# aicip/Cross-Scale-MAE

Measured on AMD Instinct MI355X. Metric: pretrain images/sec ViT-B/16 224^2 two-scale, higher is better.
Workload: dtype bf16; 1 GPU; MAE_ViT_MsLdCeCd ViT-B/16, 224^2 two-scale crops, mask 0.75, AdamW, full optimizer step; loss=mse, batch_per_gpu=128, global_batch=128, parallelism=dp1, headline_config=True

## Files before the change

### cross-scale-mae_amd/csrc/attention.hip

```cpp
#include "common.h"
#include <cstdlib>

#define LOG2E 1.4426950408889634f
#define LN2 0.6931471805599453f

template <int HD> struct AttnLds { static constexpr int STRIDE = (HD + 8) * 2; };

template <int HD, int TP>
__device__ __forceinline__ void stage_head(char* dst, const bf16_t* src, long long row0, int ld, int col0, int T, int hd) {
  constexpr int CH = HD / 8;
  for (int e = threadIdx.x; e < TP * CH; e += blockDim.x) {
    int r = e / CH, c = e - r * CH;
    uint4 v = make_uint4(0, 0, 0, 0);
    if (r < T && c * 8 < hd) v = *reinterpret_cast<const uint4*>(src + (row0 + r) * ld + col0 + c * 8);
    *reinterpret_cast<uint4*>(dst + r * AttnLds<HD>::STRIDE + c * 16) = v;
  }
}

template <int HD, int TP, int NT, int NM>
struct HeadStager {
  static constexpr int CH = HD / 8, IT = (TP * CH + NT - 1) / NT;
  uint4 v[NM][IT];
  __device__ __forceinline__ void load(int m, const bf16_t* src, long long row0, int ld, int col0, int T, int hd) {
#pragma unroll
    for (int i = 0; i < IT; ++i) {
      const int e = threadIdx.x + i * NT, r = e / CH, c = e - r * CH;
      v[m][i] = make_uint4(0, 0, 0, 0);
      if (e < TP * CH && r < T && c * 8 < hd) v[m][i] = *reinterpret_cast<const uint4*>(src + (row0 + r) * ld + col0 + c * 8);
    }
  }
  __device__ __forceinline__ void store(int m, char* dst) {
#pragma unroll
    for (int i = 0; i < IT; ++i) {
      const int e = threadIdx.x + i * NT, r = e / CH, c = e - r * CH;
      if (e < TP * CH) *reinterpret_cast<uint4*>(dst + r * AttnLds<HD>::STRIDE + c * 16) = v[m][i];
    }
  }
};

template <int HD>
__device__ __forceinline__ s8_t frag_rows(const char* img, int row0, int ks, int t, int g) {
  return *reinterpret_cast<const s8_t*>(img + (row0 + t) * AttnLds<HD>::STRIDE + (ks * 32 + 8 * g) * 2);
}
template <int HD>
__device__ __forceinline__ s8_t frag_cols_tr(const char* img, int r0, int c0, int t, int g) {
  const char* p = img + (r0 + 4 * g + (t >> 2)) * AttnLds<HD>::STRIDE + (c0 + (t & 3) * 4) * 2;
  s4_t lo = __builtin_amdgcn_ds_read_tr16_b64_v4i16(LDS_PTR(s4_t, p));
  s4_t hi = __builtin_amdgcn_ds_read_tr16_b64_v4i16(LDS_PTR(s4_t, p + 16 * AttnLds<HD>::STRIDE));
  return join_s4(lo, hi);
}
__device__ __forceinline__ s8_t pack_pair(f4_t a, f4_t b) {
  unsigned u0 = pack2bf(a[0], a[1]), u1 = pack2bf(a[2], a[3]), u2 = pack2bf(b[0], b[1]), u3 = pack2bf(b[2], b[3]);
  uint4 u = make_uint4(u0, u1, u2, u3);
  return __builtin_bit_cast(s8_t, u);
}
#define MFMA16(a, b, c) __builtin_amdgcn_mfma_f32_16x16x32_bf16(__builtin_bit_cast(bf8_t, a), __builtin_bit_cast(bf8_t, b), c, 0, 0, 0)

template <int HD>
__device__ __forceinline__ int pair_remap(int bid, int nblk) {
  if (HD * 2 >= 128 || (bid | 15) >= nblk) return bid;
  return (bid & ~15) + 2 * (bid & 7) + ((bid >> 3) & 1);
}

template <int HD, int NKF, bool EMIT = false>
__global__ __launch_bounds__(256) void attn_fwd_bf16(const bf16_t* __restrict__ qkv, bf16_t* __restrict__ out,
                                                     float* __restrict__ lse, int T, int H, int D, int hd, float scale, Fp8Emit em) {
  constexpr int TP = NKF * 16, KS = HD / 32, DF = HD / 16;
  constexpr int QB = (NKF + 3) / 4;
  __shared__ __attribute__((aligned(16))) char smem[2 * TP * AttnLds<HD>::STRIDE];
  char* Ks = smem;
  char* Vs = smem + TP * AttnLds<HD>::STRIDE;
  const int wid = pair_remap<HD>(blockIdx.x, gridDim.x);
  const int b = wid / H, h = wid - b * H;
  const long long row0 = (long long)b * T;
  const int ld = 3 * D;
  const int lane = threadIdx.x & 63, w = threadIdx.x >> 6, t = lane & 15, g = lane >> 4;
  uint4 qraw[QB][KS];
  {
    HeadStager<HD, TP, 256, 2> sg;
    sg.load(0, qkv, row0, ld, D + h * hd, T, hd); sg.load(1, qkv, row0, ld, 2 * D + h * hd, T, hd);
#pragma unroll
    for (int bq = 0; bq < QB; ++bq)
#pragma unroll
      for (int ks = 0; ks < KS; ++ks) {
        const int qr = (w + 4 * bq) * 16 + t, col = ks * 32 + 8 * g;
        qraw[bq][ks] = make_uint4(0, 0, 0, 0);
        if (qr < T && col < hd) qraw[bq][ks] = *reinterpret_cast<const uint4*>(qkv + (row0 + qr) * ld + h * hd + col);
      }
    sg.store(0, Ks); sg.store(1, Vs);
// ... 6 lines not shown
  constexpr int FIRST_PARTIAL = NKF <= 2 ? 0 : (NKF <= 6 ? NKF - 2 : (NKF == 14 ? 6 : 14));
  const int kthr = T - 4 * g;
#pragma unroll
  for (int bq = 0; bq < QB; ++bq) {
    const int qb = w + 4 * bq;
    if (qb >= nqb) break;
    const int q = qb * 16 + t;
    s8_t fq[KS];
#pragma unroll
    for (int ks = 0; ks < KS; ++ks) fq[ks] = __builtin_bit_cast(s8_t, qraw[bq][ks]);
    f4_t s[NKF];
    float m = -INFINITY;
#pragma unroll
    for (int f = 0; f < NKF; ++f) {
      f4_t a = {0.f, 0.f, 0.f, 0.f};
#pragma unroll
      for (int ks = 0; ks < KS; ++ks) a = MFMA16(frag_rows<HD>(Ks, f * 16, ks, t, g), fq[ks], a);
      if (f >= FIRST_PARTIAL) {
#pragma unroll
        for (int r = 0; r < 4; ++r) a[r] = (f * 16 + r >= kthr) ? -INFINITY : a[r];
      }
      m = fmaxf(fmaxf(m, fmaxf(a[0], a[1])), fmaxf(a[2], a[3]));
      s[f] = a;
    }
    m = xrow_max(m);
    m *= c2;
    float l = 0.f;
#pragma unroll
    for (int f = 0; f < NKF; ++f)
#pragma unroll
      for (int r = 0; r < 4; ++r) { float p = __builtin_amdgcn_exp2f(fmaf(s[f][r], c2, -m)); s[f][r] = p; l += p; }
    l = xrow_sum(l);
    const float inv = 1.0f / l;
    s8_t fp[NKF / 2];
#pragma unroll
    for (int s2 = 0; s2 < NKF / 2; ++s2) fp[s2] = pack_pair(s[2 * s2], s[2 * s2 + 1]);
#pragma unroll
    for (int df = 0; df < DF; ++df) {
      f4_t o = {0.f, 0.f, 0.f, 0.f};
#pragma unroll
      for (int s2 = 0; s2 < NKF / 2; ++s2) o = MFMA16(frag_cols_tr<HD>(Vs, 32 * s2, df * 16, t, g), fp[s2], o);
      int d = df * 16 + 4 * g;
      if (q < T && d < hd) {
        const long long at = (row0 + q) * D + h * hd + d;
        st4<bf16_t>(out + at, o * inv);
        if (EMIT) *reinterpret_cast<unsigned*>(em.q + at) = fp8_pack4(round4<bf16_t>(o * inv), qs, qmax, em.fmt, qseen);
      }
    }
    if (g == 0 && q < T) lse[((long long)b * H + h) * T + q] = (m + log2f(l)) * LN2;
  }
  if (EMIT) fp8_emit_amax(em, qseen, threadIdx.x & 63);
}

template <bool EMIT>
__device__ __forceinline__ void st4_dqkv(bf16_t* dqkv, long long at, f4_t v, const Fp8Emit& em, float qs, float qmax, float& qseen) {
  if (!EMIT || dqkv) st4<bf16_t>(dqkv + at, v);
  if (EMIT) *reinterpret_cast<unsigned*>(em.q + at) = fp8_pack4(round4<bf16_t>(v), qs, qmax, em.fmt, qseen);
}
template <int HD, int NKF, bool EMIT = false>
__global__ __launch_bounds__(256) void attn_bwd_bf16(const bf16_t* __restrict__ qkv, const bf16_t* __restrict__ out,
                                                     const bf16_t* __restrict__ dout, const float* __restrict__ lse,
                                                     bf16_t* __restrict__ dqkv, int T, int H, int D, int hd, float scale, Fp8Emit em) {
  constexpr int TP = NKF * 16, KS = HD / 32, DF = HD / 16, IMG = TP * AttnLds<HD>::STRIDE;
  __shared__ __attribute__((aligned(16))) char smem[4 * IMG + 2 * TP * 4];
  char* Qs = smem; char* Ks = smem + IMG; char* Vs = smem + 2 * IMG; char* Gs = smem + 3 * IMG;
  float* lse2 = reinterpret_cast<float*>(smem + 4 * IMG);
  float* dl = lse2 + TP;
  const int wid = pair_remap<HD>(blockIdx.x, gridDim.x);
  const int b = wid / H, h = wid - b * H;
  const long long row0 = (long long)b * T;
  const int ld = 3 * D;
  {
    HeadStager<HD, TP, 256, 4> sg;
    sg.load(0, qkv, row0, ld, h * hd, T, hd); sg.load(1, qkv, row0, ld, D + h * hd, T, hd);
    sg.load(2, qkv, row0, ld, 2 * D + h * hd, T, hd); sg.load(3, dout, row0, D, h * hd, T, hd);
    sg.store(0, Qs); sg.store(1, Ks); sg.store(2, Vs); sg.store(3, Gs);
  }
  for (int r = threadIdx.x; r < TP; r += blockDim.x) {
    float acc = 0.f, l2 = INFINITY;
    if (r < T) {
      l2 = lse[((long long)b * H + h) * T + r] * LOG2E;
      const bf16_t* o = out + (row0 + r) * D + h * hd;
      const bf16_t* gg = dout + (row0 + r) * D + h * hd;
      uint4 ov[HD / 8], gv[HD / 8];
#pragma unroll
      for (int c = 0; c < HD / 8; ++c) {
        ov[c] = c * 8 < hd ? *reinterpret_cast<const uint4*>(o + c * 8) : make_uint4(0, 0, 0, 0);
        gv[c] = c * 8 < hd ? *reinterpret_cast<const uint4*>(gg + c * 8) : make_uint4(0, 0, 0, 0);
      }
#pragma unroll
      for (int c = 0; c < HD / 8; ++c) {
        const unsigned ow[4] = {ov[c].x, ov[c].y, ov[c].z, ov[c].w}, gw[4] = {gv[c].x, gv[c].y, gv[c].z, gv[c].w};
#pragma unroll
        for (int k = 0; k < 4; ++k)
          acc += __uint_as_float(ow[k] << 16) * __uint_as_float(gw[k] << 16) + __uint_as_float(ow[k] & 0xffff0000u) * __uint_as_float(gw[k] & 0xffff0000u);
      }
    }
    lse2[r] = l2; dl[r] = acc;
  }
  __syncthreads();
  const int lane = threadIdx.x & 63, w = threadIdx.x >> 6, t = lane & 15, g = lane >> 4;
  float qmax = 0.f, qseen = 0.f;
  const float qs = EMIT ? fp8_emit_scale(em, lane, qmax) : 1.f;
  const float c2 = scale * LOG2E;
  const int nblk = (T + 15) >> 4;
  for (int qb = w; qb < nblk; qb += 4) {
    const int q = qb * 16 + t;
    s8_t fq[KS], fg[KS];
#pragma unroll
    for (int ks = 0; ks < KS; ++ks) { fq[ks] = frag_rows<HD>(Qs, qb * 16, ks, t, g); fg[ks] = frag_rows<HD>(Gs, qb * 16, ks, t, g); }
    const float my_l2 = lse2[q], my_dl = dl[q];
    s8_t fds[NKF / 2];
    f4_t prev = {0.f, 0.f, 0.f, 0.f};
#pragma unroll
    for (int f = 0; f < NKF; ++f) {
      f4_t a = {0.f, 0.f, 0.f, 0.f}, dp = {0.f, 0.f, 0.f, 0.f};
#pragma unroll
      for (int ks = 0; ks < KS; ++ks) {
        a = MFMA16(frag_rows<HD>(Ks, f * 16, ks, t, g), fq[ks], a);
        dp = MFMA16(frag_rows<HD>(Vs, f * 16, ks, t, g), fg[ks], dp);
      }
      f4_t ds;
#pragma unroll
      for (int r = 0; r < 4; ++r) {
        float p = __builtin_amdgcn_exp2f(a[r] * c2 - my_l2);
        ds[r] = p * (dp[r] - my_dl) * scale;
      }
      if (f & 1) fds[f >> 1] = pack_pair(prev, ds); else prev = ds;
    }
#pragma unroll
    for (int df = 0; df < DF; ++df) {
      f4_t o = {0.f, 0.f, 0.f, 0.f};
#pragma unroll
      for (int s2 = 0; s2 < NKF / 2; ++s2) o = MFMA16(frag_cols_tr<HD>(Ks, 32 * s2, df * 16, t, g), fds[s2], o);
      int d = df * 16 + 4 * g;
      if (q < T && d < hd) st4_dqkv<EMIT>(dqkv, (row0 + q) * ld + h * hd + d, o, em, qs, qmax, qseen);
    }
  }
  for (int kb = w; kb < nblk; kb += 4) {
    const int key = kb * 16 + t;
    s8_t fk[KS], fv[KS];
#pragma unroll
    for (int ks = 0; ks < KS; ++ks) { fk[ks] = frag_rows<HD>(Ks, kb * 16, ks, t, g); fv[ks] = frag_rows<HD>(Vs, kb * 16, ks, t, g); }
    s8_t fp[NKF / 2], fds[NKF / 2];
    f4_t prev_p = {0.f, 0.f, 0.f, 0.f}, prev_ds = {0.f, 0.f, 0.f, 0.f};
#pragma unroll
    for (int f = 0; f < NKF; ++f) {
      f4_t a = {0.f, 0.f, 0.f, 0.f}, dp = {0.f, 0.f, 0.f, 0.f};
#pragma unroll
      for (int ks = 0; ks < KS; ++ks) {
        a = MFMA16(frag_rows<HD>(Qs, f * 16, ks, t, g), fk[ks], a);
        dp = MFMA16(frag_rows<HD>(Gs, f * 16, ks, t, g), fv[ks], dp);
      }
      f4_t l4 = *reinterpret_cast<const f4_t*>(lse2 + f * 16 + 4 * g);
      f4_t d4 = *reinterpret_cast<const f4_t*>(dl + f * 16 + 4 * g);
      f4_t p, ds;
#pragma unroll
      for (int r = 0; r < 4; ++r) {
        p[r] = __builtin_amdgcn_exp2f(a[r] * c2 - l4[r]);
        ds[r] = p[r] * (dp[r] - d4[r]) * scale;
      }
      if (f & 1) { fp[f >> 1] = pack_pair(prev_p, p); fds[f >> 1] = pack_pair(prev_ds, ds); } else { prev_p = p; prev_ds = ds; }
    }
#pragma unroll
    for (int df = 0; df < DF; ++df) {
      f4_t ok = {0.f, 0.f, 0.f, 0.f}, ov = {0.f, 0.f, 0.f, 0.f};
#pragma unroll
      for (int s2 = 0; s2 < NKF / 2; ++s2) {
        ok = MFMA16(frag_cols_tr<HD>(Qs, 32 * s2, df * 16, t, g), fds[s2], ok);
        ov = MFMA16(frag_cols_tr<HD>(Gs, 32 * s2, df * 16, t, g), fp[s2], ov);
      }
      int d = df * 16 + 4 * g;
      if (key < T && d < hd) {
        st4_dqkv<EMIT>(dqkv, (row0 + key) * ld + D + h * hd + d, ok, em, qs, qmax, qseen);
        st4_dqkv<EMIT>(dqkv, (row0 + key) * ld + 2 * D + h * hd + d, ov, em, qs, qmax, qseen);
      }
    }
  }
  if (EMIT) fp8_emit_amax(em, qseen, lane);
}

template <int HD, int NKF>
struct AttnBwd1p {
  static constexpr int NP = NKF / 2, TP = NKF * 16, IMG = TP * AttnLds<HD>::STRIDE, QS = HD + 4;
  static constexpr int XB = 32 * HD * 2;
  static constexpr int LDS = 2 * IMG + TP * QS * 4 + 4 * XB + 2 * TP * 4;
  static constexpr int LDS8 = LDS + 4 * XB;
};
template <int HD>
__device__ __forceinline__ s8_t patch_cols_tr(const char* img, int c0, int t, int g) {
  const char* p = img + (4 * g + (t >> 2)) * (HD * 2) + (c0 + (t & 3) * 4) * 2;
  s4_t lo = __builtin_amdgcn_ds_read_tr16_b64_v4i16(LDS_PTR(s4_t, p));
  s4_t hi = __builtin_amdgcn_ds_read_tr16_b64_v4i16(LDS_PTR(s4_t, p + 16 * HD * 2));
  return join_s4(lo, hi);
}
#ifdef ATTN_TIMING
__device__ unsigned long long g_attn_ts[16];
extern "C" int csmae_debug_attn_ts(unsigned long long* out) { return (int)hipMemcpyFromSymbol(out, HIP_SYMBOL(g_attn_ts), sizeof(g_attn_ts)); }
#define TS(i) do { if (blockIdx.x == 300 && threadIdx.x == 0) g_attn_ts[i] = __builtin_readcyclecounter(); } while (0)
#else
#define TS(i)
#endif
template <int HD, int NKF, bool EMIT = false, int NW = 4>
__global__ __launch_bounds__(NW * 64, NW == 4 ? 2 : 1) void attn_bwd1p_bf16(const bf16_t* __restrict__ qkv, const bf16_t* __restrict__ out,
                                                           const bf16_t* __restrict__ dout, const float* __restrict__ lse,
                                                           bf16_t* __restrict__ dqkv, int T, int H, int D, int hd, float scale, Fp8Emit em) {
  using L = AttnBwd1p<HD, NKF>;
  constexpr int TP = L::TP, NP = L::NP, KS = HD / 32, DF = HD / 16, IMG = L::IMG, QS = L::QS;
  static_assert(NW == 4 || (NW == 8 && NP >= 8), "eight waves need at least eight query pairs for the dQ rotation");
  __shared__ __attribute__((aligned(16))) char smem[NW == 4 ? L::LDS : L::LDS8];
  char* Qs = smem; char* Gs = smem + IMG;
  float* dqa = reinterpret_cast<float*>(smem + 2 * IMG);
  char* xall = smem + 2 * IMG + TP * QS * 4;
  float* lse2 = reinterpret_cast<float*>(xall + NW * L::XB);
  float* dl = lse2 + TP;
  const int wid = pair_remap<HD>(blockIdx.x, gridDim.x);
  const int b = wid / H, h = wid - b * H;
  const long long row0 = (long long)b * T;
  const int ld = 3 * D;
  const int lane = threadIdx.x & 63, w = threadIdx.x >> 6, t = lane & 15, g = lane >> 4;
  float qmax = 0.f, qseen = 0.f;
  const float qs = EMIT ? fp8_emit_scale(em, lane, qmax) : 1.f;
  TS(0);
  HeadStager<HD, TP, NW * 64, 2> sg;
  sg.load(0, qkv, row0, ld, h * hd, T, hd); sg.load(1, dout, row0, D, h * hd, T, hd);
  const int nkp = (T + 31) >> 5;
  uint4 kraw[2][KS], vraw[2][KS];
  auto load_kv = [&](int kp) {
#pragma unroll
    for (int jj = 0; jj < 2; ++jj)
#pragma unroll
      for (int ks = 0; ks < KS; ++ks) {
        const int key = 32 * kp + 16 * jj + t, col = ks * 32 + 8 * g;
        kraw[jj][ks] = make_uint4(0, 0, 0, 0); vraw[jj][ks] = make_uint4(0, 0, 0, 0);
        if (kp < nkp && key < T && col < hd) {
          kraw[jj][ks] = *reinterpret_cast<const uint4*>(qkv + (row0 + key) * ld + D + h * hd + col);
          vraw[jj][ks] = *reinterpret_cast<const uint4*>(qkv + (row0 + key) * ld + 2 * D + h * hd + col);
        }
      }
  };
  load_kv(w);
  for (int e = threadIdx.x; e < TP * QS / 4; e += blockDim.x) reinterpret_cast<f4_t*>(dqa)[e] = f4_t{0.f, 0.f, 0.f, 0.f};
  for (int r = threadIdx.x; r < TP; r += blockDim.x) {
    float acc = 0.f, l2 = INFINITY;
    if (r < T) {
      l2 = lse[((long long)b * H + h) * T + r] * LOG2E;
      const bf16_t* o = out + (row0 + r) * D + h * hd;
      const bf16_t* gg = dout + (row0 + r) * D + h * hd;
      uint4 ov[HD / 8], gv[HD / 8];
#pragma unroll
      for (int c = 0; c < HD / 8; ++c) {
        ov[c] = c * 8 < hd ? *reinterpret_cast<const uint4*>(o + c * 8) : make_uint4(0, 0, 0, 0);
        gv[c] = c * 8 < hd ? *reinterpret_cast<const uint4*>(gg + c * 8) : make_uint4(0, 0, 0, 0);
      }
#pragma unroll
      for (int c = 0; c < HD / 8; ++c) {
        const unsigned ow[4] = {ov[c].x, ov[c].y, ov[c].z, ov[c].w}, gw[4] = {gv[c].x, gv[c].y, gv[c].z, gv[c].w};
#pragma unroll
        for (int k = 0; k < 4; ++k)
          acc += __uint_as_float(ow[k] << 16) * __uint_as_float(gw[k] << 16) + __uint_as_float(ow[k] & 0xffff0000u) * __uint_as_float(gw[k] & 0xffff0000u);
      }
    }
    lse2[r] = l2; dl[r] = acc;
  }
  TS(1);
  sg.store(0, Qs); sg.store(1, Gs);
  const float c2 = scale * LOG2E;
  char* xw = xall + w * L::XB;
  const int nq = (T + 31) >> 5;
  for (int sweep = 0; sweep * NW < nkp; ++sweep) {
    const int kp = sweep * NW + w;
    const bool active = kp < nkp;
    const int k0 = 32 * kp;
    s8_t fk[2][KS], fv[2][KS], kT[DF];
#pragma unroll
    for (int jj = 0; jj < 2; ++jj)
#pragma unroll
      for (int ks = 0; ks < KS; ++ks) {
        const int col = ks * 32 + 8 * g;
        fk[jj][ks] = __builtin_bit_cast(s8_t, kraw[jj][ks]); fv[jj][ks] = __builtin_bit_cast(s8_t, vraw[jj][ks]);
        *reinterpret_cast<uint4*>(xw + (16 * jj + t) * (HD * 2) + col * 2) = kraw[jj][ks];
      }
#pragma unroll
    for (int df = 0; df < DF; ++df) kT[df] = patch_cols_tr<HD>(xw, df * 16, t, g);
    f4_t dk[2][DF], dv[2][DF];
#pragma unroll
    for (int jj = 0; jj < 2; ++jj)
#pragma unroll
      for (int df = 0; df < DF; ++df) { dk[jj][df] = f4_t{0.f, 0.f, 0.f, 0.f}; dv[jj][df] = f4_t{0.f, 0.f, 0.f, 0.f}; }
    TS(2 + 4 * sweep);
    __syncthreads();
    TS(3 + 4 * sweep);
    if ((sweep + 1) * NW < nkp) load_kv((sweep + 1) * NW + w);
    for (int s = 0; s < nq; ++s) {
      int ip = w + s; if (ip >= nq) ip -= nq;
      const int q0 = 32 * ip;
      if (active && w < nq) {
        f4_t p[2][2], ds[2][2];
#pragma unroll
        for (int ii = 0; ii < 2; ++ii) {
          s8_t fq[KS], fg[KS];
#pragma unroll
          for (int ks = 0; ks < KS; ++ks) { fq[ks] = frag_rows<HD>(Qs, q0 + 16 * ii, ks, t, g); fg[ks] = frag_rows<HD>(Gs, q0 + 16 * ii, ks, t, g); }
          const f4_t l4 = *reinterpret_cast<const f4_t*>(lse2 + q0 + 16 * ii + 4 * g);
          const f4_t d4 = *reinterpret_cast<const f4_t*>(dl + q0 + 16 * ii + 4 * g);
#pragma unroll
          for (int jj = 0; jj < 2; ++jj) {
            f4_t a = {0.f, 0.f, 0.f, 0.f}, dp = {0.f, 0.f, 0.f, 0.f};
#pragma unroll
            for (int ks = 0; ks < KS; ++ks) { a = MFMA16(fq[ks], fk[jj][ks], a); dp = MFMA16(fg[ks], fv[jj][ks], dp); }
#pragma unroll
            for (int r = 0; r < 4; ++r) {
              p[ii][jj][r] = __builtin_amdgcn_exp2f(a[r] * c2 - l4[r]);
              ds[ii][jj][r] = p[ii][jj][r] * (dp[r] - d4[r]) * scale;
            }
            uint2 u = make_uint2(pack2bf(ds[ii][jj][0], ds[ii][jj][1]), pack2bf(ds[ii][jj][2], ds[ii][jj][3]));
            *reinterpret_cast<uint2*>(xw + (ii * 2 + jj) * 512 + t * 32 + g * 8) = u;
          }
        }
// ... 15 lines not shown
          f4_t* dst = reinterpret_cast<f4_t*>(dqa + (q0 + 16 * ii + t) * QS + 4 * g);
#pragma unroll
          for (int df = 0; df < DF; ++df) dst[df * 4] = MFMA16(kT[df], sT, dst[df * 4]);
        }
      }
      __syncthreads();
    }
    TS(4 + 4 * sweep);
    if (active) {
#pragma unroll
      for (int jj = 0; jj < 2; ++jj) {
        const int key = k0 + 16 * jj + t;
#pragma unroll
        for (int df = 0; df < DF; ++df) {
          const int d = df * 16 + 4 * g;
          if (key < T && d < hd) {
            st4_dqkv<EMIT>(dqkv, (row0 + key) * ld + D + h * hd + d, dk[jj][df], em, qs, qmax, qseen);
            st4_dqkv<EMIT>(dqkv, (row0 + key) * ld + 2 * D + h * hd + d, dv[jj][df], em, qs, qmax, qseen);
          }
        }
      }
    }
  }
  TS(10);
  for (int e = threadIdx.x; e < T * (HD / 4); e += blockDim.x) {
    const int q = e / (HD / 4), d = (e - q * (HD / 4)) * 4;
    if (d < hd) st4_dqkv<EMIT>(dqkv, (row0 + q) * ld + h * hd + d, *reinterpret_cast<const f4_t*>(dqa + q * QS + d), em, qs, qmax, qseen);
  }
  if (EMIT) fp8_emit_amax(em, qseen, lane);
}

template <int HD, int NKF, bool EMIT = false>
__global__ __launch_bounds__(256, 2) void attn_bwd1p2_bf16(const bf16_t* __restrict__ qkv, const bf16_t* __restrict__ out,
                                                            const bf16_t* __restrict__ dout, const float* __restrict__ lse,
                                                            bf16_t* __restrict__ dqkv, int T, int H, int D, int hd, float scale, Fp8Emit em) {
  using L = AttnBwd1p<HD, NKF>;
  constexpr int TP = L::TP, NP = L::NP, KS = HD / 32, DF = HD / 16, IMG = L::IMG, QS = L::QS;
  static_assert(NP <= 8, "two key pairs per wave cover at most eight");
  constexpr int NPW = NP > 4 ? 2 : 1;
  __shared__ __attribute__((aligned(16))) char smem[L::LDS];
  char* Qs = smem; char* Gs = smem + IMG;
  float* dqa = reinterpret_cast<float*>(smem + 2 * IMG);
  char* xall = smem + 2 * IMG + TP * QS * 4;
  float* lse2 = reinterpret_cast<float*>(xall + 4 * L::XB);
  float* dl = lse2 + TP;
  const int wid = pair_remap<HD>(blockIdx.x, gridDim.x);
  const int b = wid / H, h = wid - b * H;
  const long long row0 = (long long)b * T;
  const int ld = 3 * D;
  const int lane = threadIdx.x & 63, w = threadIdx.x >> 6, t = lane & 15, g = lane >> 4;
  float qmax = 0.f, qseen = 0.f;
  const float qs = EMIT ? fp8_emit_scale(em, lane, qmax) : 1.f;
  TS(0);
  HeadStager<HD, TP, 256, 2> sg;
  sg.load(0, qkv, row0, ld, h * hd, T, hd); sg.load(1, dout, row0, D, h * hd, T, hd);
  const int nkp = (T + 31) >> 5;
  uint4 kraw[NPW][2][KS], vraw[NPW][2][KS];
#pragma unroll
  for (int pi = 0; pi < NPW; ++pi)
#pragma unroll
    for (int jj = 0; jj < 2; ++jj)
#pragma unroll
      for (int ks = 0; ks < KS; ++ks) {
        const int kp = w + 4 * pi, key = 32 * kp + 16 * jj + t, col = ks * 32 + 8 * g;
        kraw[pi][jj][ks] = make_uint4(0, 0, 0, 0); vraw[pi][jj][ks] = make_uint4(0, 0, 0, 0);
        if (kp < nkp && key < T && col < hd) {
          kraw[pi][jj][ks] = *reinterpret_cast<const uint4*>(qkv + (row0 + key) * ld + D + h * hd + col);
          vraw[pi][jj][ks] = *reinterpret_cast<const uint4*>(qkv + (row0 + key) * ld + 2 * D + h * hd + col);
        }
      }
  for (int e = threadIdx.x; e < TP * QS / 4; e += blockDim.x) reinterpret_cast<f4_t*>(dqa)[e] = f4_t{0.f, 0.f, 0.f, 0.f};
  for (int r = threadIdx.x; r < TP; r += blockDim.x) {
    float acc = 0.f, l2 = INFINITY;
    if (r < T) {
      l2 = lse[((long long)b * H + h) * T + r] * LOG2E;
      const bf16_t* o = out + (row0 + r) * D + h * hd;
      const bf16_t* gg = dout + (row0 + r) * D + h * hd;
      uint4 ov[HD / 8], gv[HD / 8];
#pragma unroll
      for (int c = 0; c < HD / 8; ++c) {
        ov[c] = c * 8 < hd ? *reinterpret_cast<const uint4*>(o + c * 8) : make_uint4(0, 0, 0, 0);
        gv[c] = c * 8 < hd ? *reinterpret_cast<const uint4*>(gg + c * 8) : make_uint4(0, 0, 0, 0);
      }
#pragma unroll
      for (int c = 0; c < HD / 8; ++c) {
        const unsigned ow[4] = {ov[c].x, ov[c].y, ov[c].z, ov[c].w}, gw[4] = {gv[c].x, gv[c].y, gv[c].z, gv[c].w};
#pragma unroll
        for (int k = 0; k < 4; ++k)
          acc += __uint_as_float(ow[k] << 16) * __uint_as_float(gw[k] << 16) + __uint_as_float(ow[k] & 0xffff0000u) * __uint_as_float(gw[k] & 0xffff0000u);
      }
    }
    lse2[r] = l2; dl[r] = acc;
  }
  TS(1);
  sg.store(0, Qs); sg.store(1, Gs);
  const float c2 = scale * LOG2E;
  char* xw = xall + w * L::XB;
  const int nq = (T + 31) >> 5;
  const bool act0 = w < nkp, act1 = w + 4 < nkp;
  s8_t fk[NPW][2][KS], fv[NPW][2][KS], kT[NPW][DF];
  f4_t dk[NPW][2][DF], dv[NPW][2][DF];
#pragma unroll
  for (int pi = 0; pi < NPW; ++pi) {
#pragma unroll
    for (int jj = 0; jj < 2; ++jj)
#pragma unroll
      for (int ks = 0; ks < KS; ++ks) {
        const int col = ks * 32 + 8 * g;
        fk[pi][jj][ks] = __builtin_bit_cast(s8_t, kraw[pi][jj][ks]); fv[pi][jj][ks] = __builtin_bit_cast(s8_t, vraw[pi][jj][ks]);
        *reinterpret_cast<uint4*>(xw + (16 * jj + t) * (HD * 2) + col * 2) = kraw[pi][jj][ks];
      }
#pragma unroll
    for (int df = 0; df < DF; ++df) kT[pi][df] = patch_cols_tr<HD>(xw, df * 16, t, g);
#pragma unroll
    for (int jj = 0; jj < 2; ++jj)
#pragma unroll
      for (int df = 0; df < DF; ++df) { dk[pi][jj][df] = f4_t{0.f, 0.f, 0.f, 0.f}; dv[pi][jj][df] = f4_t{0.f, 0.f, 0.f, 0.f}; }
  }
  TS(2);
  __syncthreads();
  TS(3);
  for (int s = 0; s < nq; ++s) {
    int ip = w + s; if (ip >= nq) ip -= nq;
    const int q0 = 32 * ip;
    if (act0) {
      s8_t fq[2][KS], fg[2][KS], qT[DF], gT[DF];
      f4_t l4[2], d4[2], dq[2][DF];
#pragma unroll
      for (int ii = 0; ii < 2; ++ii) {
#pragma unroll
        for (int ks = 0; ks < KS; ++ks) { fq[ii][ks] = frag_rows<HD>(Qs, q0 + 16 * ii, ks, t, g); fg[ii][ks] = frag_rows<HD>(Gs, q0 + 16 * ii, ks, t, g); }
        l4[ii] = *reinterpret_cast<const f4_t*>(lse2 + q0 + 16 * ii + 4 * g);
        d4[ii] = *reinterpret_cast<const f4_t*>(dl + q0 + 16 * ii + 4 * g);
#pragma unroll
        for (int df = 0; df < DF; ++df) dq[ii][df] = f4_t{0.f, 0.f, 0.f, 0.f};
      }
#pragma unroll
      for (int df = 0; df < DF; ++df) { qT[df] = frag_cols_tr<HD>(Qs, q0, df * 16, t, g); gT[df] = frag_cols_tr<HD>(Gs, q0, df * 16, t, g); }
#pragma unroll
      for (int pi = 0; pi < NPW; ++pi) {
        if (pi == 1 && !act1) continue;
        uint2 pp[2][2], dsp[2][2];
#pragma unroll
        for (int ii = 0; ii < 2; ++ii)
#pragma unroll
          for (int jj = 0; jj < 2; ++jj) {
            f4_t a = {0.f, 0.f, 0.f, 0.f}, dp = {0.f, 0.f, 0.f, 0.f};
#pragma unroll
            for (int ks = 0; ks < KS; ++ks) { a = MFMA16(fq[ii][ks], fk[pi][jj][ks], a); dp = MFMA16(fg[ii][ks], fv[pi][jj][ks], dp); }
            f4_t p, ds;
#pragma unroll
            for (int r = 0; r < 4; ++r) {
              p[r] = __builtin_amdgcn_exp2f(a[r] * c2 - l4[ii][r]);
              ds[r] = p[r] * (dp[r] - d4[ii][r]) * scale;
            }
            pp[ii][jj] = make_uint2(pack2bf(p[0], p[1]), pack2bf(p[2], p[3]));
            const uint2 u = make_uint2(pack2bf(ds[0], ds[1]), pack2bf(ds[2], ds[3]));
            dsp[ii][jj] = u;
            *reinterpret_cast<uint2*>(xw + (ii * 2 + jj) * 512 + t * 32 + g * 8) = u;
          }
#pragma unroll
        for (int df = 0; df < DF; ++df)
#pragma unroll
          for (int jj = 0; jj < 2; ++jj) {
            dk[pi][jj][df] = MFMA16(qT[df], __builtin_bit_cast(s8_t, make_uint4(dsp[0][jj].x, dsp[0][jj].y, dsp[1][jj].x, dsp[1][jj].y)), dk[pi][jj][df]);
            dv[pi][jj][df] = MFMA16(gT[df], __builtin_bit_cast(s8_t, make_uint4(pp[0][jj].x, pp[0][jj].y, pp[1][jj].x, pp[1][jj].y)), dv[pi][jj][df]);
          }
#pragma unroll
        for (int ii = 0; ii < 2; ++ii) {
          const char* xp = xw + ii * 1024 + (4 * g + (t >> 2)) * 32 + (t & 3) * 8;
          s4_t lo = __builtin_amdgcn_ds_read_tr16_b64_v4i16(LDS_PTR(s4_t, xp));
          s4_t hi = __builtin_amdgcn_ds_read_tr16_b64_v4i16(LDS_PTR(s4_t, xp + 512));
          const s8_t sT = join_s4(lo, hi);
#pragma unroll
          for (int df = 0; df < DF; ++df) dq[ii][df] = MFMA16(kT[pi][df], sT, dq[ii][df]);
        }
      }
#pragma unroll
      for (int ii = 0; ii < 2; ++ii) {
        f4_t* dst = reinterpret_cast<f4_t*>(dqa + (q0 + 16 * ii + t) * QS + 4 * g);
#pragma unroll
        for (int df = 0; df < DF; ++df) dst[df * 4] += dq[ii][df];
      }
    }
    __syncthreads();
    if (s == 0) TS(5);
  }
  TS(4);
#pragma unroll
  for (int pi = 0; pi < NPW; ++pi) {
#pragma unroll
    for (int jj = 0; jj < 2; ++jj) {
      const int key = 32 * (w + 4 * pi) + 16 * jj + t;
#pragma unroll
      for (int df = 0; df < DF; ++df) {
        const int d = df * 16 + 4 * g;
        if (key < T && d < hd) {
          st4_dqkv<EMIT>(dqkv, (row0 + key) * ld + D + h * hd + d, dk[pi][jj][df], em, qs, qmax, qseen);
          st4_dqkv<EMIT>(dqkv, (row0 + key) * ld + 2 * D + h * hd + d, dv[pi][jj][df], em, qs, qmax, qseen);
        }
      }
    }
  }
  TS(10);
  for (int e = threadIdx.x; e < T * (HD / 4); e += blockDim.x) {
    const int q = e / (HD / 4), d = (e - q * (HD / 4)) * 4;
    if (d < hd) st4_dqkv<EMIT>(dqkv, (row0 + q) * ld + h * hd + d, *reinterpret_cast<const f4_t*>(dqa + q * QS + d), em, qs, qmax, qseen);
  }
  TS(11);
  if (EMIT) fp8_emit_amax(em, qseen, lane);
}

template <int HD>
__global__ __launch_bounds__(256) void attn_fwd_f32(const float* __restrict__ qkv, float* __restrict__ out,
                                                    float* __restrict__ lse, int T, int H, int D, int hd, float scale) {
  extern __shared__ float sm[];
  const int S = hd + 1;
  float* Ks = sm; float* Vs = sm + T * S;
  const int b = blockIdx.x / H, h = blockIdx.x - b * H;
  const long long row0 = (long long)b * T;
  const int ld = 3 * D;
  for (int e = threadIdx.x; e < T * hd; e += blockDim.x) {
    int r = e / hd, d = e - r * hd;
    Ks[r * S + d] = qkv[(row0 + r) * ld + D + h * hd + d];
    Vs[r * S + d] = qkv[(row0 + r) * ld + 2 * D + h * hd + d];
  }
  __syncthreads();
  for (int q = threadIdx.x; q < T; q += blockDim.x) {
    float qr[HD];
#pragma unroll
    for (int d = 0; d < HD; ++d) qr[d] = d < hd ? qkv[(row0 + q) * ld + h * hd + d] * scale : 0.f;
    float m = -INFINITY;
    for (int j = 0; j < T; ++j) {
      float s = 0.f;
#pragma unroll
      for (int d = 0; d < HD; ++d) if (d < hd) s = fmaf(qr[d], Ks[j * S + d], s);
      m = fmaxf(m, s);
// ... 146 lines not shown
#pragma unroll
    for (int d = 0; d < HD; ++d) dq[d] = 0.f;
    const float lq = ls[q], dlq = dl[q];
    for (int j = 0; j < Tn; ++j) {
      const T* kr = qkv + (row0 + j) * ld + D + h * hd;
      const float ds = expf(dot(qi, kr) * scale - lq) * (dot(gi, kr + D) - dlq) * scale;
      axpy(dq, ds, kr);
    }
    store_row(dq, dqkv + (row0 + q) * ld + h * hd);
  }
  for (int j = threadIdx.x; j < Tn; j += blockDim.x) {
    float kj[HD], vj[HD], dk[HD], dv[HD];
    load_row(kj, qkv + (row0 + j) * ld + D + h * hd); load_row(vj, qkv + (row0 + j) * ld + 2 * D + h * hd);
#pragma unroll
    for (int d = 0; d < HD; ++d) { dk[d] = 0.f; dv[d] = 0.f; }
    for (int i = 0; i < Tn; ++i) {
      const T* qr = qkv + (row0 + i) * ld + h * hd;
      const T* gr = dout + (row0 + i) * D + h * hd;
      const float pij = expf(dot(kj, qr) * scale - ls[i]);
      const float ds = pij * (dot(vj, gr) - dl[i]) * scale;
      axpy(dk, ds, qr); axpy(dv, pij, gr);
    }
    store_row(dk, dqkv + (row0 + j) * ld + D + h * hd);
    store_row(dv, dqkv + (row0 + j) * ld + 2 * D + h * hd);
  }
}
template <typename T>
static void launch_any(bool bwd, long long B, int Tn, int H, int D, int hd, float scale, const void* qkv, const void* out, const void* dout, float* lse_w, const float* lse_r,
                       void* o, hipStream_t st) {
  const int BH = (int)(B * H);
#define ANY(HDV)                                                                                                                                     \
  if (!bwd) hipLaunchKernelGGL((attn_fwd_any<T, HDV>), dim3(cdiv(Tn, 256), BH), dim3(256), 0, st, (const T*)qkv, (T*)o, lse_w, Tn, H, D, hd, scale);   \
  else hipLaunchKernelGGL((attn_bwd_any<T, HDV>), dim3(BH), dim3(256), (size_t)2 * Tn * sizeof(float), st, (const T*)qkv, (const T*)out, (const T*)dout, lse_r, (T*)o, Tn, H, D, hd, scale)
  if (hd <= 32) { ANY(32); } else if (hd <= 64) { ANY(64); } else if (hd <= 96) { ANY(96); } else { ANY(128); }
#undef ANY
}

template <int HD, int NKF>
static void launch_fwd_bf16(int BH, const void* qkv, void* out, float* lse, int T, int H, int D, int hd, float scale, hipStream_t st, const Fp8Emit* em) {
  if (em) hipLaunchKernelGGL((attn_fwd_bf16<HD, NKF, true>), dim3(BH), dim3(256), 0, st, (const bf16_t*)qkv, (bf16_t*)out, lse, T, H, D, hd, scale, *em);
  else hipLaunchKernelGGL((attn_fwd_bf16<HD, NKF, false>), dim3(BH), dim3(256), 0, st, (const bf16_t*)qkv, (bf16_t*)out, lse, T, H, D, hd, scale, Fp8Emit{});
}
template <int HD, int NKF>
static void launch_bwd_bf16(int BH, const void* qkv, const void* out, const void* dout, const float* lse, void* dqkv, int T, int H, int D, int hd, float scale, hipStream_t st,
                            const Fp8Emit* em) {
  static const bool two_pass = csmae_debug_opt("attn_bwd_2pass") != nullptr;
  static const bool two_sweeps = csmae_debug_opt("attn_bwd_2sweep") != nullptr;
  constexpr bool KP2_OK = HD <= 32 && NKF >= 6 && NKF <= 16 && AttnBwd1p<HD, NKF>::LDS <= 160 * 1024;
  constexpr int NK1 = AttnBwd1p<HD, NKF>::LDS <= 160 * 1024 ? NKF : 2;
  constexpr bool W8_OK = NKF >= 18 && AttnBwd1p<HD, NKF>::LDS8 <= 160 * 1024;
  static const bool four_waves = csmae_debug_opt("attn_bwd_4waves") != nullptr;
#define ATTN_BWD_ARGS (const bf16_t*)qkv, (const bf16_t*)out, (const bf16_t*)dout, lse, (bf16_t*)dqkv, T, H, D, hd, scale
  if (KP2_OK && !two_pass && !two_sweeps) {
    if (em) CSMAE_LAUNCH((attn_bwd1p2_bf16<HD, (KP2_OK ? NKF : 2), true>), dim3(BH), dim3(256), 0, st, ATTN_BWD_ARGS, *em);
    else CSMAE_LAUNCH((attn_bwd1p2_bf16<HD, (KP2_OK ? NKF : 2), false>), dim3(BH), dim3(256), 0, st, ATTN_BWD_ARGS, Fp8Emit{});
  } else if (W8_OK && !two_pass && !four_waves) {
    if constexpr (W8_OK) {
      if (em) CSMAE_LAUNCH((attn_bwd1p_bf16<HD, NKF, true, 8>), dim3(BH), dim3(512), 0, st, ATTN_BWD_ARGS, *em);
      else CSMAE_LAUNCH((attn_bwd1p_bf16<HD, NKF, false, 8>), dim3(BH), dim3(512), 0, st, ATTN_BWD_ARGS, Fp8Emit{});
    }
  } else if (AttnBwd1p<HD, NKF>::LDS <= 160 * 1024 && NKF >= 6 && !two_pass) {
    if (em) CSMAE_LAUNCH((attn_bwd1p_bf16<HD, NK1, true>), dim3(BH), dim3(256), 0, st, ATTN_BWD_ARGS, *em);
    else CSMAE_LAUNCH((attn_bwd1p_bf16<HD, NK1, false>), dim3(BH), dim3(256), 0, st, ATTN_BWD_ARGS, Fp8Emit{});
  } else {
    if (em) CSMAE_LAUNCH((attn_bwd_bf16<HD, NKF, true>), dim3(BH), dim3(256), 0, st, ATTN_BWD_ARGS, *em);
    else CSMAE_LAUNCH((attn_bwd_bf16<HD, NKF, false>), dim3(BH), dim3(256), 0, st, ATTN_BWD_ARGS, Fp8Emit{});
  }
#undef ATTN_BWD_ARGS
}

#define NKF_SMALL(HDV, CALL)                                 \
  if (T <= 32) { CALL(HDV, 2); }                             \
  else if (T <= 64) { CALL(HDV, 4); }                        \
  else if (T <= 96) { CALL(HDV, 6); }
#define DISPATCH_BF16(CALL)                                                            \
  if (hd <= 32) { NKF_SMALL(32, CALL) else if (T <= 224) { CALL(32, 14); } else { CALL(32, 18); } } \
  else if (hd <= 64) { NKF_SMALL(64, CALL) else { CALL(64, 14); } }                    \
  else { NKF_SMALL(96, CALL) }

static bool bf16_resident(int T, int hd) { return hd % 8 == 0 && T <= 288 && (hd <= 32 || (hd <= 64 && T <= 224) || (hd <= 96 && T <= 96)); }
static int check_common(const char* who, long long B, int T, int H, int D, int hd) {
  CSMAE_REQUIRE(B > 0 && T > 0 && H > 0 && hd > 0 && D == H * hd, "%s: bad geometry B=%lld T=%d H=%d D=%d hd=%d", who, B, T, H, D, hd);
  CSMAE_REQUIRE(hd <= 128 && hd % 4 == 0 && T <= 8192 && B * H <= 0x7fffffffll, "%s: head_dim %d (multiple of 4, <= 128) / sequence length %d (<= 8192) unsupported", who, hd, T);
  return CSMAE_OK;
}

static int attn_fwd_impl(int dtype, long long B, int T, int H, int hd, const void* qkv, void* out, float* lse, void* stream, const Fp8Emit* em) {
  const int D = H * hd;
  int rc = check_common("csmae_attn_fwd", B, T, H, D, hd);
  if (rc) return rc;
  hipStream_t st = (hipStream_t)stream;
  const float scale = 1.0f / sqrtf((float)hd);
  const int BH = (int)(B * H);
  if (dtype == CSMAE_BF16) {
    if (!bf16_resident(T, hd)) { CSMAE_REQUIRE(!em, "csmae_attn_fwd_q: the fp8 copy is emitted by the LDS-resident kernels only (csmae_attn_resident)"); launch_any<bf16_t>(false, B, T, H, D, hd, scale, qkv, nullptr, nullptr, lse, nullptr, out, st); return csmae_check_launch("csmae_attn_fwd"); }
#define CALLF(HDV, NK) launch_fwd_bf16<HDV, NK>(BH, qkv, out, lse, T, H, D, hd, scale, st, em)
    DISPATCH_BF16(CALLF)
#undef CALLF
  } else if (dtype == CSMAE_F32) {
    size_t sh = (size_t)2 * T * (hd + 1) * sizeof(float);
    if (sh > 160 * 1024 || hd > 96) { launch_any<float>(false, B, T, H, D, hd, scale, qkv, nullptr, nullptr, lse, nullptr, out, st); return csmae_check_launch("csmae_attn_fwd"); }
    if (hd <= 32) hipLaunchKernelGGL((attn_fwd_f32<32>), dim3(BH), dim3(256), sh, st, (const float*)qkv, (float*)out, lse, T, H, D, hd, scale);
    else if (hd <= 64) hipLaunchKernelGGL((attn_fwd_f32<64>), dim3(BH), dim3(256), sh, st, (const float*)qkv, (float*)out, lse, T, H, D, hd, scale);
    else hipLaunchKernelGGL((attn_fwd_f32<96>), dim3(BH), dim3(256), sh, st, (const float*)qkv, (float*)out, lse, T, H, D, hd, scale);
  } else { csmae_set_error("csmae_attn_fwd: unsupported dtype %d", dtype); return CSMAE_ERR_UNSUPPORTED; }
  return csmae_check_launch("csmae_attn_fwd");
}

// ... 51 lines not shown
```

Baseline: 6170 images/s.

## Fuse row-delta computation into Q/dO staging and defer LDS landing across sweeps

Attention backward kernels now load Q, dO, O and the lse row together in a single register stager. Each thread computes its chunk of the O·dO dot product and reduces across chunks with DPP, so out and dout are no longer re-read by a separate per-row loop. In the bwd1p2 kernel, part of the staged Q/dO is written to LDS before the first barrier, and the rest is written inside later sweep iterations to overlap with compute. The cost is more live registers and reliance on the compiler scheduling hints. The timing macros are moved earlier so the base kernel can use them.

```diff
diff --git a/cross-scale-mae_amd/csrc/attention.hip b/cross-scale-mae_amd/csrc/attention.hip
--- a/cross-scale-mae_amd/csrc/attention.hip
+++ b/cross-scale-mae_amd/csrc/attention.hip
@@ -35,6 +35,73 @@
       const int e = threadIdx.x + i * NT, r = e / CH, c = e - r * CH;
       if (e < TP * CH) *reinterpret_cast<uint4*>(dst + r * AttnLds<HD>::STRIDE + c * 16) = v[m][i];
     }
+  }
+};
+
+__device__ __forceinline__ float delta_chunk(float acc, uint4 o, uint4 g) {
+  const unsigned ow[4] = {o.x, o.y, o.z, o.w}, gw[4] = {g.x, g.y, g.z, g.w};
+#pragma unroll
+  for (int k = 0; k < 4; ++k)
+    acc += __uint_as_float(ow[k] << 16) * __uint_as_float(gw[k] << 16) + __uint_as_float(ow[k] & 0xffff0000u) * __uint_as_float(gw[k] & 0xffff0000u);
+  return acc;
+}
+template <int HD, int TP>
+__device__ __forceinline__ void row_stats_global(float* lse2, float* dl, const bf16_t* out, const bf16_t* dout, const float* lrow, long long row0, int D, int col0, int T, int hd) {
+  for (int r = threadIdx.x; r < TP; r += blockDim.x) {
+    float acc = 0.f, l2 = INFINITY;
+    if (r < T) {
+      l2 = lrow[r] * LOG2E;
+      const bf16_t* o = out + (row0 + r) * D + col0;
+      const bf16_t* gg = dout + (row0 + r) * D + col0;
+      uint4 ov[HD / 8], gv[HD / 8];
+#pragma unroll
+      for (int c = 0; c < HD / 8; ++c) {
+        ov[c] = c * 8 < hd ? *reinterpret_cast<const uint4*>(o + c * 8) : make_uint4(0, 0, 0, 0);
+        gv[c] = c * 8 < hd ? *reinterpret_cast<const uint4*>(gg + c * 8) : make_uint4(0, 0, 0, 0);
+      }
+#pragma unroll
+      for (int c = 0; c < HD / 8; ++c) acc = delta_chunk(acc, ov[c], gv[c]);
+    }
+    lse2[r] = l2; dl[r] = acc;
+  }
+}
+
+template <int HD, int TP, int NT>
+struct RowStager {
+  static constexpr int CH = HD / 8, IT = (TP * CH + NT - 1) / NT;
+  static constexpr bool OK = (CH & (CH - 1)) == 0 && CH <= 16;
+  uint4 q[IT], g[IT], o[IT];
+  float l[IT];
+  static constexpr int its_for_pair(int p) { return (32 * (p + 1) * CH + NT - 1) / NT < IT ? (32 * (p + 1) * CH + NT - 1) / NT : IT; }
+  __device__ __forceinline__ void load(const bf16_t* qkv, const bf16_t* out, const bf16_t* dout, const float* lrow, long long row0, int ld, int D, int col0, int T, int hd) {
+#pragma unroll
+    for (int i = 0; i < IT; ++i) {
+      const int e = threadIdx.x + i * NT, r = e / CH, c = e - r * CH;
+      const int rc = r < T ? r : T - 1, cc = c * 8 < hd ? c * 8 : 0;
+      q[i] = *reinterpret_cast<const uint4*>(qkv + (row0 + rc) * ld + col0 + cc);
+      g[i] = *reinterpret_cast<const uint4*>(dout + (row0 + rc) * D + col0 + cc);
+      o[i] = *reinterpret_cast<const uint4*>(out + (row0 + rc) * D + col0 + cc);
+      l[i] = lrow[rc];
+      __builtin_amdgcn_sched_barrier(0);
+    }
+  }
+  __device__ __forceinline__ void pin(int i) {
+    asm volatile("" : "+v"(q[i].x), "+v"(q[i].y), "+v"(q[i].z), "+v"(q[i].w), "+v"(g[i].x), "+v"(g[i].y), "+v"(g[i].z), "+v"(g[i].w),
+                      "+v"(o[i].x), "+v"(o[i].y), "+v"(o[i].z), "+v"(o[i].w), "+v"(l[i]));
+  }
+  __device__ __forceinline__ void land(int i, char* Qs, char* Gs, float* lse2, float* dl, int T, int hd) {
+    const int e = threadIdx.x + i * NT, r = e / CH, c = e - r * CH;
+    const bool live = r < T && c * 8 < hd;
+    const uint4 z = make_uint4(0, 0, 0, 0), qv = live ? q[i] : z, gv = live ? g[i] : z, ov = live ? o[i] : z;
+    if (e < TP * CH) {
+      *reinterpret_cast<uint4*>(Qs + r * AttnLds<HD>::STRIDE + c * 16) = qv;
+      *reinterpret_cast<uint4*>(Gs + r * AttnLds<HD>::STRIDE + c * 16) = gv;
+    }
+    float acc = delta_chunk(0.f, ov, gv);
+#pragma unroll
+    for (int j = 1; j < CH; ++j)
+      acc = delta_chunk(__builtin_bit_cast(float, __builtin_amdgcn_update_dpp(0, __builtin_bit_cast(int, acc), 0x111, 0xf, 0xf, false)), ov, gv);
+    if (e < TP * CH && c == CH - 1) { lse2[r] = r < T ? l[i] * LOG2E : INFINITY; dl[r] = acc; }
   }
 };
 
@@ -147,6 +214,13 @@
   if (EMIT) fp8_emit_amax(em, qseen, threadIdx.x & 63);
 }
 
+#ifdef ATTN_TIMING
+__device__ unsigned long long g_attn_ts[16];
+extern "C" int csmae_debug_attn_ts(unsigned long long* out) { return (int)hipMemcpyFromSymbol(out, HIP_SYMBOL(g_attn_ts), sizeof(g_attn_ts)); }
+#define TS(i) do { if (blockIdx.x == 300 && threadIdx.x == 0) g_attn_ts[i] = __builtin_readcyclecounter(); } while (0)
+#else
+#define TS(i)
+#endif
 template <bool EMIT>
 __device__ __forceinline__ void st4_dqkv(bf16_t* dqkv, long long at, f4_t v, const Fp8Emit& em, float qs, float qmax, float& qseen) {
   if (!EMIT || dqkv) st4<bf16_t>(dqkv + at, v);
@@ -165,35 +239,17 @@
   const int b = wid / H, h = wid - b * H;
   const long long row0 = (long long)b * T;
   const int ld = 3 * D;
+  TS(0);
   {
     HeadStager<HD, TP, 256, 4> sg;
     sg.load(0, qkv, row0, ld, h * hd, T, hd); sg.load(1, qkv, row0, ld, D + h * hd, T, hd);
     sg.load(2, qkv, row0, ld, 2 * D + h * hd, T, hd); sg.load(3, dout, row0, D, h * hd, T, hd);
     sg.store(0, Qs); sg.store(1, Ks); sg.store(2, Vs); sg.store(3, Gs);
   }
-  for (int r = threadIdx.x; r < TP; r += blockDim.x) {
-    float acc = 0.f, l2 = INFINITY;
-    if (r < T) {
-      l2 = lse[((long long)b * H + h) * T + r] * LOG2E;
-      const bf16_t* o = out + (row0 + r) * D + h * hd;
-      const bf16_t* gg = dout + (row0 + r) * D + h * hd;
-      uint4 ov[HD / 8], gv[HD / 8];
-#pragma unroll
-      for (int c = 0; c < HD / 8; ++c) {
-        ov[c] = c * 8 < hd ? *reinterpret_cast<const uint4*>(o + c * 8) : make_uint4(0, 0, 0, 0);
-        gv[c] = c * 8 < hd ? *reinterpret_cast<const uint4*>(gg + c * 8) : make_uint4(0, 0, 0, 0);
-      }
-#pragma unroll
-      for (int c = 0; c < HD / 8; ++c) {
-        const unsigned ow[4] = {ov[c].x, ov[c].y, ov[c].z, ov[c].w}, gw[4] = {gv[c].x, gv[c].y, gv[c].z, gv[c].w};
-#pragma unroll
-        for (int k = 0; k < 4; ++k)
-          acc += __uint_as_float(ow[k] << 16) * __uint_as_float(gw[k] << 16) + __uint_as_float(ow[k] & 0xffff0000u) * __uint_as_float(gw[k] & 0xffff0000u);
-      }
-    }
-    lse2[r] = l2; dl[r] = acc;
-  }
+  row_stats_global<HD, TP>(lse2, dl, out, dout, lse + ((long long)b * H + h) * T, row0, D, h * hd, T, hd);
+  TS(2);
   __syncthreads();
+  TS(3);
   const int lane = threadIdx.x & 63, w = threadIdx.x >> 6, t = lane & 15, g = lane >> 4;
   float qmax = 0.f, qseen = 0.f;
   const float qs = EMIT ? fp8_emit_scale(em, lane, qmax) : 1.f;
@@ -232,6 +288,7 @@
       if (q < T && d < hd) st4_dqkv<EMIT>(dqkv, (row0 + q) * ld + h * hd + d, o, em, qs, qmax, qseen);
     }
   }
+  TS(4);
   for (int kb = w; kb < nblk; kb += 4) {
     const int key = kb * 16 + t;
     s8_t fk[KS], fv[KS];
@@ -272,6 +329,7 @@
       }
     }
   }
+  TS(11);
   if (EMIT) fp8_emit_amax(em, qseen, lane);
 }
 
@@ -289,13 +347,6 @@
   s4_t hi = __builtin_amdgcn_ds_read_tr16_b64_v4i16(LDS_PTR(s4_t, p + 16 * HD * 2));
   return join_s4(lo, hi);
 }
-#ifdef ATTN_TIMING
-__device__ unsigned long long g_attn_ts[16];
-extern "C" int csmae_debug_attn_ts(unsigned long long* out) { return (int)hipMemcpyFromSymbol(out, HIP_SYMBOL(g_attn_ts), sizeof(g_attn_ts)); }
-#define TS(i) do { if (blockIdx.x == 300 && threadIdx.x == 0) g_attn_ts[i] = __builtin_readcyclecounter(); } while (0)
-#else
-#define TS(i)
-#endif
 template <int HD, int NKF, bool EMIT = false, int NW = 4>
 __global__ __launch_bounds__(NW * 64, NW == 4 ? 2 : 1) void attn_bwd1p_bf16(const bf16_t* __restrict__ qkv, const bf16_t* __restrict__ out,
                                                            const bf16_t* __restrict__ dout, const float* __restrict__ lse,
@@ -317,8 +368,6 @@
   float qmax = 0.f, qseen = 0.f;
   const float qs = EMIT ? fp8_emit_scale(em, lane, qmax) : 1.f;
   TS(0);
-  HeadStager<HD, TP, NW * 64, 2> sg;
-  sg.load(0, qkv, row0, ld, h * hd, T, hd); sg.load(1, dout, row0, D, h * hd, T, hd);
   const int nkp = (T + 31) >> 5;
   uint4 kraw[2][KS], vraw[2][KS];
   auto load_kv = [&](int kp) {
@@ -335,31 +384,21 @@
       }
   };
   load_kv(w);
+  using RS = RowStager<HD, TP, NW * 64>;
+  RS rs;
+  HeadStager<HD, TP, NW * 64, 2> sg;
+  const float* lrow = lse + ((long long)b * H + h) * T;
+  if constexpr (RS::OK) rs.load(qkv, out, dout, lrow, row0, ld, D, h * hd, T, hd);
+  else { sg.load(0, qkv, row0, ld, h * hd, T, hd); sg.load(1, dout, row0, D, h * hd, T, hd); }
   for (int e = threadIdx.x; e < TP * QS / 4; e += blockDim.x) reinterpret_cast<f4_t*>(dqa)[e] = f4_t{0.f, 0.f, 0.f, 0.f};
-  for (int r = threadIdx.x; r < TP; r += blockDim.x) {
-    float acc = 0.f, l2 = INFINITY;
-    if (r < T) {
-      l2 = lse[((long long)b * H + h) * T + r] * LOG2E;
-      const bf16_t* o = out + (row0 + r) * D + h * hd;
-      const bf16_t* gg = dout + (row0 + r) * D + h * hd;
-      uint4 ov[HD / 8], gv[HD / 8];
-#pragma unroll
-      for (int c = 0; c < HD / 8; ++c) {
-        ov[c] = c * 8 < hd ? *reinterpret_cast<const uint4*>(o + c * 8) : make_uint4(0, 0, 0, 0);
-        gv[c] = c * 8 < hd ? *reinterpret_cast<const uint4*>(gg + c * 8) : make_uint4(0, 0, 0, 0);
-      }
-#pragma unroll
-      for (int c = 0; c < HD / 8; ++c) {
-        const unsigned ow[4] = {ov[c].x, ov[c].y, ov[c].z, ov[c].w}, gw[4] = {gv[c].x, gv[c].y, gv[c].z, gv[c].w};
-#pragma unroll
-        for (int k = 0; k < 4; ++k)
-          acc += __uint_as_float(ow[k] << 16) * __uint_as_float(gw[k] << 16) + __uint_as_float(ow[k] & 0xffff0000u) * __uint_as_float(gw[k] & 0xffff0000u);
-      }
-    }
-    lse2[r] = l2; dl[r] = acc;
-  }
   TS(1);
-  sg.store(0, Qs); sg.store(1, Gs);
+  if constexpr (RS::OK) {
+#pragma unroll
+    for (int i = 0; i < RS::IT; ++i) rs.land(i, Qs, Gs, lse2, dl, T, hd);
+  } else {
+    row_stats_global<HD, TP>(lse2, dl, out, dout, lrow, row0, D, h * hd, T, hd);
+    sg.store(0, Qs); sg.store(1, Gs);
+  }
   const float c2 = scale * LOG2E;
   char* xw = xall + w * L::XB;
   const int nq = (T + 31) >> 5;
@@ -481,8 +520,9 @@
   float qmax = 0.f, qseen = 0.f;
   const float qs = EMIT ? fp8_emit_scale(em, lane, qmax) : 1.f;
   TS(0);
-  HeadStager<HD, TP, 256, 2> sg;
-  sg.load(0, qkv, row0, ld, h * hd, T, hd); sg.load(1, dout, row0, D, h * hd, T, hd);
+  using RS = RowStager<HD, TP, 256>;
+  static_assert(RS::OK, "head_dim 32: four chunks per row");
+  RS rs;
   const int nkp = (T + 31) >> 5;
   uint4 kraw[NPW][2][KS], vraw[NPW][2][KS];
 #pragma unroll
@@ -498,31 +538,10 @@
           vraw[pi][jj][ks] = *reinterpret_cast<const uint4*>(qkv + (row0 + key) * ld + 2 * D + h * hd + col);
         }
       }
+  __builtin_amdgcn_sched_barrier(0);
+  rs.load(qkv, out, dout, lse + ((long long)b * H + h) * T, row0, ld, D, h * hd, T, hd);
   for (int e = threadIdx.x; e < TP * QS / 4; e += blockDim.x) reinterpret_cast<f4_t*>(dqa)[e] = f4_t{0.f, 0.f, 0.f, 0.f};
-  for (int r = threadIdx.x; r < TP; r += blockDim.x) {
-    float acc = 0.f, l2 = INFINITY;
-    if (r < T) {
-      l2 = lse[((long long)b * H + h) * T + r] * LOG2E;
-      const bf16_t* o = out + (row0 + r) * D + h * hd;
-      const bf16_t* gg = dout + (row0 + r) * D + h * hd;
-      uint4 ov[HD / 8], gv[HD / 8];
-#pragma unroll
-      for (int c = 0; c < HD / 8; ++c) {
-        ov[c] = c * 8 < hd ? *reinterpret_cast<const uint4*>(o + c * 8) : make_uint4(0, 0, 0, 0);
-        gv[c] = c * 8 < hd ? *reinterpret_cast<const uint4*>(gg + c * 8) : make_uint4(0, 0, 0, 0);
-      }
-#pragma unroll
-      for (int c = 0; c < HD / 8; ++c) {
-        const unsigned ow[4] = {ov[c].x, ov[c].y, ov[c].z, ov[c].w}, gw[4] = {gv[c].x, gv[c].y, gv[c].z, gv[c].w};
-#pragma unroll
-        for (int k = 0; k < 4; ++k)
-          acc += __uint_as_float(ow[k] << 16) * __uint_as_float(gw[k] << 16) + __uint_as_float(ow[k] & 0xffff0000u) * __uint_as_float(gw[k] & 0xffff0000u);
-      }
-    }
-    lse2[r] = l2; dl[r] = acc;
-  }
   TS(1);
-  sg.store(0, Qs); sg.store(1, Gs);
   const float c2 = scale * LOG2E;
   char* xw = xall + w * L::XB;
   const int nq = (T + 31) >> 5;
@@ -546,6 +565,9 @@
 #pragma unroll
       for (int df = 0; df < DF; ++df) { dk[pi][jj][df] = f4_t{0.f, 0.f, 0.f, 0.f}; dv[pi][jj][df] = f4_t{0.f, 0.f, 0.f, 0.f}; }
   }
+  constexpr int PAIRS0 = NP < 4 ? NP : 4;
+#pragma unroll
+  for (int i = 0; i < RS::its_for_pair(PAIRS0 - 1); ++i) rs.land(i, Qs, Gs, lse2, dl, T, hd);
   TS(2);
   __syncthreads();
   TS(3);
@@ -612,6 +634,12 @@
         for (int df = 0; df < DF; ++df) dst[df * 4] += dq[ii][df];
       }
     }
+#pragma unroll
+    for (int k = 0; k + PAIRS0 < NP; ++k)
+      if (s == k) {
+#pragma unroll
+        for (int i = RS::its_for_pair(k + PAIRS0 - 1); i < RS::its_for_pair(k + PAIRS0); ++i) { rs.pin(i); rs.land(i, Qs, Gs, lse2, dl, T, hd); }
+      }
     __syncthreads();
     if (s == 0) TS(5);
   }
@@ -864,8 +892,8 @@
   static const bool four_waves = csmae_debug_opt("attn_bwd_4waves") != nullptr;
 #define ATTN_BWD_ARGS (const bf16_t*)qkv, (const bf16_t*)out, (const bf16_t*)dout, lse, (bf16_t*)dqkv, T, H, D, hd, scale
   if (KP2_OK && !two_pass && !two_sweeps) {
-    if (em) CSMAE_LAUNCH((attn_bwd1p2_bf16<HD, (KP2_OK ? NKF : 2), true>), dim3(BH), dim3(256), 0, st, ATTN_BWD_ARGS, *em);
-    else CSMAE_LAUNCH((attn_bwd1p2_bf16<HD, (KP2_OK ? NKF : 2), false>), dim3(BH), dim3(256), 0, st, ATTN_BWD_ARGS, Fp8Emit{});
+    if (em) CSMAE_LAUNCH((attn_bwd1p2_bf16<(KP2_OK ? HD : 32), (KP2_OK ? NKF : 2), true>), dim3(BH), dim3(256), 0, st, ATTN_BWD_ARGS, *em);
+    else CSMAE_LAUNCH((attn_bwd1p2_bf16<(KP2_OK ? HD : 32), (KP2_OK ? NKF : 2), false>), dim3(BH), dim3(256), 0, st, ATTN_BWD_ARGS, Fp8Emit{});
   } else if (W8_OK && !two_pass && !four_waves) {
     if constexpr (W8_OK) {
       if (em) CSMAE_LAUNCH((attn_bwd1p_bf16<HD, NKF, true, 8>), dim3(BH), dim3(512), 0, st, ATTN_BWD_ARGS, *em);
```

After: 6179 images/s (median of 4 runs). Within noise of the previous version (+0.2%).
